# QingYunA/General-Medical-Image-Segmentation-CNN-Framework

Measured on AMD Instinct MI355X. Metric: train voxels/sec (128^3 patches) 3D U-Net, higher is better.
Workload: dtype f32 (f16x3 split MFMA: every fp32 conv operand = two fp16 parts under a per-tensor power-of-two scale, three fp16 products per fp32 product, fp32 accumulate; graded against fp64 by the same tests as bf16x6 and the exact-fp32 MFMA path); 1 GPU; unet3d_f32_2x128: UNet3D(1,2,32) fwd+BCE+bwd+Adam+Dice, x=[2,1,128,128,128] fp32 per GPU, random-init (kaiming) weights, data-parallel replicas with RCCL gradient all-reduce, conv math f16x3; global_batch=2, parallelism=dp1, conv_math=f16x3, optimizer=torch.optim.Adam(fused=True)

## Files before the change

### general-medical-image-segmentation-cnn-framework_amd/csrc/conv_bf16_api.hip

```cpp
#include "common.h"
#include "internal.h"
#include "igemm_kernel.h"

namespace seg {

template <typename TS, typename TD>
__global__ __launch_bounds__(256) void cast_rows_kernel(const TS* __restrict__ src, int lds, TD* __restrict__ dst, int ldd, long long rows, int C) {
    const bool v = (C % 4 == 0) && (lds % 4 == 0) && (ldd % 4 == 0) && ((uintptr_t)src % (4 * sizeof(TS)) == 0) && ((uintptr_t)dst % (4 * sizeof(TD)) == 0);
    const int cw = v ? C / 4 : C;
    const long long total = rows * cw;
    for (long long i = (long long)blockIdx.x * blockDim.x + threadIdx.x; i < total; i += (long long)gridDim.x * blockDim.x) {
        const long long r = i / cw;
        const int c = (int)(i - r * cw);
        if (v) st4(dst + r * ldd + c * 4, ld4(src + r * lds + c * 4));
        else st1(dst + r * ldd + c, ld1(src + r * lds + c));
    }
}

template <typename TS, typename TD>
static void cast_rows(const TS* src, int lds, TD* dst, int ldd, long long rows, int C, hipStream_t st) {
    long long b = (rows * C / 4 + 255) / 256;
    const int grid = (int)(b < 1 ? 1 : (b > 8192 ? 8192 : b));
    hipLaunchKernelGGL((cast_rows_kernel<TS, TD>), dim3(grid), dim3(256), 0, st, src, lds, dst, ldd, rows, C);
}
// ... 35 lines not shown
    {NB_CAST, RUNG(headk_wgrad_supported(SHAPE5(g), g.Cin, g.Cout))},
    {NB_TINY, RUNG(tinypw_supported(SHAPE5(g)))},
    {NB_PWL, RUNG(pointwise(g) && pw_wgrad_lowp_supported(conv_vin(g), g.Cin, g.Cout, k.ldx, k.ldy, 2)), WS(pw_wgrad_lowp_ws_bytes(conv_vin(g), g.Cin, g.Cout)), pointwise, al16, NB_PW},
    {NB_PW, RUNG(pointwise(g) && pw_wgrad_supported(conv_vin(g), g.Cin, g.Cout, 1, k.ldx, k.ldy)), nullptr, nullptr, al8},
    {NB_STEM4, RUNG(stem4_lowp_supported(SHAPE5(g), k.ldx, k.ldy)), ws_stem4, nullptr, al16, NB_STEM},
    {NB_STEM, RUNG(stem_supported(SHAPE5(g), k.ldy)), nullptr, nullptr, al8},
    {NB_HEADPW, RUNG(headpw_lowp_supported(SHAPE5(g), k.ldx, k.ldy)), ws_headpw, nullptr, al16, NB_HEAD},
    {NB_HEAD, RUNG(head_supported(SHAPE5(g), k.ldx)), nullptr, nullptr, al8},
    {NB_SMALLCIN, RUNG(smallcin_wgrad_supported(g.Cin, g.Cout, g.k)), nullptr, nullptr, al8},
    {NB_SMALLCOUT, RUNG(smallcout_wgrad_supported(g.Cin, g.Cout, g.k, k.ldx)), nullptr, nullptr, al8},
    {NB_GW, RUNG(gwgrad_supported(GEOM9(g), k.ldx, k.ldy)), nullptr, nullptr, al8},
    {NB_CAST}};
static int choose_b16(const Rung* r, const ConvKey& k) {
    while (r->fits && !r->fits(k)) ++r;
    if (!r->aligned || r->aligned(k)) return r->family;
    for (const Rung* d = r + 1; r->demote && d->fits; ++d)
        if (d->family == r->demote) return d->fits(k) && d->aligned(k) ? d->family : NB_CAST;
    return NB_CAST;
}

template <typename F>
static int staged(const ConvCall& c, bool x_in, bool y_in, F run) {
    const ConvGeom& g = c.g;
    Carver cv(c.ws);
    float* xf = cv.take<float>((size_t)c.vin() * g.Cin);
    float* yf = cv.take<float>((size_t)c.vout() * g.Cout);
    const size_t used = cv.used();
    SEG_CHECK_WS(used + mi355seg_conv3d_ws_bytes(GEOM9(g)), c.ws_bytes);
    if (x_in) cast_rows((const bf16*)c.x, c.ldx, xf, g.Cin, c.vin(), g.Cin, c.st);
    if (y_in) cast_rows((const bf16*)c.y, c.ldy, yf, g.Cout, c.vout(), g.Cout, c.st);
    SEG_CHECK_LAUNCH();
    int rc = run(xf, yf, (char*)c.ws + used, c.ws_bytes - used);
    if (rc || (x_in && y_in)) return rc;
    if (x_in) cast_rows(yf, g.Cout, (bf16*)c.y, c.ldy, c.vout(), g.Cout, c.st);
    else cast_rows(xf, g.Cin, (bf16*)c.x, c.ldx, c.vin(), g.Cin, c.st);
    SEG_CHECK_LAUNCH();
    return MI355SEG_OK;
}

}

using namespace seg;

extern "C" {

int mi355seg_set_b16_tiles(int mode) {
    SEG_CHECK_ARG(mode >= 0 && mode <= 2, "set_b16_tiles: 0 (auto), 1 (16x16x32 tiles wherever possible) or 2 (generic tiles), got %d", mode);
    set_b16_tiles(mode);
    return MI355SEG_OK;
}
int mi355seg_get_b16_tiles(void) { return get_b16_tiles(); }

int mi355seg_set_wgrad_wide(int mode) {
    SEG_CHECK_ARG(mode >= 0 && mode <= 2, "set_wgrad_wide: 0 (never), 1 (where it pays) or 2 (wherever the geometry allows), got %d", mode);
    set_wgrad_wide(mode);
    return MI355SEG_OK;
}
int mi355seg_get_wgrad_wide(void) { return get_wgrad_wide(); }

size_t mi355seg_conv3d_ws_bytes_bf16(int N, int D, int H, int W, int Cin, int Cout, int k, int stride, int pad) {
    size_t base = mi355seg_conv3d_ws_bytes(N, D, H, W, Cin, Cout, k, stride, pad);
    if (D + 2 * pad < k || H + 2 * pad < k || W + 2 * pad < k) return base;
    const ConvGeom g{N, D, H, W, Cin, Cout, k, stride, pad, (D + 2 * pad - k) / stride + 1, (H + 2 * pad - k) / stride + 1, (W + 2 * pad - k) / stride + 1};
    for (const Rung* ladder : {FWD_B16, DGRAD_B16, WGRAD_B16})
        if (ladder_ws_bytes(ladder, g) > base) base = ladder_ws_bytes(ladder, g);
    const ConvKey d = dense_key(g);
    const bool fb = !choose_b16(FWD_B16, d) || !choose_b16(DGRAD_B16, d) || !choose_b16(WGRAD_B16, d);
    const size_t stage = align_up((size_t)N * D * H * W * Cin * 4, 256) + align_up((size_t)N * g.Do * g.Ho * g.Wo * Cout * 4, 256) + 512;
    if (fb || stage <= ((size_t)512 << 20)) base += stage;
    return base;
}

int mi355seg_conv3d_fused_supported_bf16(int N, int D, int H, int W, int Cin, int Cout, int k, int stride, int pad, int ldx, int ldy) {
    return choose_b16(FWD_B16, ConvKey{{N, D, H, W, Cin, Cout, k, stride, pad, 0, 0, 0}, ldx, ldy, 0, 0, 0}) == NB_IGEMM;
}
int mi355seg_conv3d_fwd_fused_bf16(const mi355seg_bf16* x, int ldx, const float* w, const float* oscale, const float* oshift, int act, float slope,
                                   mi355seg_bf16* y, int ldy, int N, int D, int H, int W, int Cin, int Cout, int k, int stride, int pad,
                                   void* ws, size_t ws_bytes, void* stream) {
    ConvCall c;
    int rc = conv_call(&c, "conv3d_fwd_fused_bf16", x, ldx, w, y, ldy, N, D, H, W, Cin, Cout, k, stride, pad, ws, ws_bytes, stream);
    if (rc) return rc;
    SEG_CHECK_ARG(oscale && oshift, "conv3d_fwd_fused_bf16: null pointer or pitch < channels");
    SEG_CHECK_ARG(choose_b16(FWD_B16, conv_key(c)) == NB_IGEMM, "conv3d_fwd_fused_bf16: no fused form for this shape / alignment (ask mi355seg_conv3d_fused_supported_bf16)");
    MfmaOpts o;
    o.oscale = oscale; o.act = act; o.slope = slope;
    return conv_fwd_mfma(MATH_B16, x, ldx, w, oshift, y, ldy, N, D, H, W, Cin, Cout, k, 0, nullptr, nullptr, ws, ws_bytes, c.st, o);
}

int mi355seg_conv3d_fwd_res_bf16(const mi355seg_bf16* x, int ldx, const float* w, const float* bias, const mi355seg_bf16* res, int ldres,
                                 mi355seg_bf16* y, int ldy, int N, int D, int H, int W, int Cin, int Cout, int k, int stride, int pad,
                                 void* ws, size_t ws_bytes, void* stream) {
    ConvCall c;
    int rc = conv_call(&c, "conv3d_fwd_res_bf16", x, ldx, w, y, ldy, N, D, H, W, Cin, Cout, k, stride, pad, ws, ws_bytes, stream);
    if (rc) return rc;
    SEG_CHECK_ARG(res && ldres >= Cout, "conv3d_fwd_res_bf16: null residual or pitch < channels");
    int fused = 0;
    if (choose_b16(FWD_B16, conv_key(c)) == NB_IGEMM) {
        MfmaOpts o;
        o.res = res; o.ldres = ldres; o.res_fused = &fused;
        rc = conv_fwd_mfma(MATH_B16, x, ldx, w, bias, y, ldy, N, D, H, W, Cin, Cout, k, 0, nullptr, nullptr, ws, ws_bytes, c.st, o);
    } else {
        rc = mi355seg_conv3d_fwd_bf16(x, ldx, w, bias, y, ldy, N, D, H, W, Cin, Cout, k, stride, pad, nullptr, nullptr, ws, ws_bytes, stream);
    }
    if (rc || fused) return rc;
    return mi355seg_act_fwd_bf16(y, ldy, res, ldres, y, ldy, c.vout(), Cout, 0, 0.f, stream);
}

int mi355seg_conv3d_fwd_bf16(const mi355seg_bf16* x, int ldx, const float* w, const float* bias, mi355seg_bf16* y, int ldy,
                             int N, int D, int H, int W, int Cin, int Cout, int k, int stride, int pad,
                             double* stats_sum, double* stats_sq, void* ws, size_t ws_bytes, void* stream) {
    ConvCall c;
// ... 115 lines not shown
```

### general-medical-image-segmentation-cnn-framework_amd/csrc/conv_wgrad_lowp.hip

```cpp
#include "common.h"
#include "internal.h"
#include <initializer_list>
#include <type_traits>
#include <stdlib.h>

namespace seg {

using f32x16 = __attribute__((ext_vector_type(16))) float;
using f32x4 = __attribute__((ext_vector_type(4))) float;
typedef short s16x4 __attribute__((ext_vector_type(4)));
typedef short s16x8 __attribute__((ext_vector_type(8)));
typedef __attribute__((address_space(3))) s16x4 lds_s16x4;

constexpr int LW_WAVES = 8;
constexpr int LW_THREADS = LW_WAVES * 64;
constexpr int LW_TPW = 4;

template <int BX, int KS, int NP, int S = 1>
struct LTile {
    static constexpr int HALO = KS / 2;
    static constexpr int NTAPS = KS == 3 ? 27 : KS * KS;
    static constexpr int PLANES = KS == 3 ? 1 : KS;
    static constexpr int VOX = (NP >= 2 || S == 2) ? 128 : 256;
    static constexpr int TY = BX == 8 ? 8 : 4;
// ... 553 lines not shown
#pragma unroll
                    for (int pr = 0; pr < NPR; ++pr)
#pragma unroll
                        for (int a2 = 0; a2 < 2; ++a2) mfma(cur, tt, a2, b, pr);
                    load_b1(b, ks + 1);
                }
#pragma unroll
                for (int k = 0; k < 4; ++k) { __builtin_amdgcn_sched_group_barrier(0x008, 2 * NPR, 0); __builtin_amdgcn_sched_group_barrier(0x100, 3 * NP, 0); }
            } else {
#pragma unroll
                for (int pr = 0; pr < NPR; ++pr)
#pragma unroll
                    for (int a2 = 0; a2 < 2; ++a2)
#pragma unroll
                        for (int b = 0; b < 4; ++b) mfma(cur, tt, a2, b, pr);
#pragma unroll
                for (int k = 0; k < 8; ++k) { __builtin_amdgcn_sched_group_barrier(0x100, 1, 0); __builtin_amdgcn_sched_group_barrier(0x008, NPR, 0); }
            }
            __builtin_amdgcn_sched_barrier(0);
        }
    };

    int tile = strip;
    tile_geom(tile, tile < a.ntiles);
#pragma unroll
    for (int j = 0; j < NPC; ++j) load_piece(j);
#pragma unroll
    for (int j = 0; j < NPC; ++j) split_piece(j);
    for (; tile < a.ntiles; tile += a.nstrips) {
        __syncthreads();
        if (!LW_DBG(a, 16) || tile == strip) write_stage();
        __syncthreads();
        tile_geom(LW_DBG(a, 64) ? strip : tile + a.nstrips, tile + a.nstrips < a.ntiles && !LW_DBG(a, 8));
        tile_mfma();
    }

#pragma unroll
    for (int tt = 0; tt < FW_TPW; ++tt) {
        const int tap = wave + FW_WAVES * tt;
        float* dst = a.part + (((long long)strip * a.ntaps_total + plane * NTAPS + tap) * a.Cin + ci0 + 4 * g) * a.Cout + co0 + li;
        if (tap <= NTAPS - 1) {
#pragma unroll
            for (int ab = 0; ab < 8; ++ab)
#pragma unroll
                for (int e = 0; e < 4; ++e) {
                    float v = acc[tt][ab >> 2][ab & 3][e];
                    if constexpr (F32) v = __builtin_ldexpf(v, -(sx + sd));
                    dst[(long long)(16 * (ab >> 2) + e) * a.Cout + 16 * (ab & 3)] = v;
                }
        }
    }
}

static int g_wgrad_wide = [] { const char* e = getenv("MI355SEG_WGRAD_WIDE"); return e ? atoi(e) : 1; }();
void set_wgrad_wide(int mode) { g_wgrad_wide = mode; }
int get_wgrad_wide() { return g_wgrad_wide; }

struct LWgradPlan { int KS, BX, ntx, nty, ntz, ntiles, nstrips, npairs, taps, planes, cob; };

static bool lwgrad_plan(int math, int KS, int stride, int N, int D, int H, int W, int Cin, int Cout, LWgradPlan* p, bool wide = false) {
    if ((KS != 3 && KS != 5) || Cin % 32 || Cout % 32 || W < 4) return false;
    if (wide && (stride != 1 || Cout % 64 || (math == MATH_X3 && KS != 3))) return false;
    if (stride != 1 && !(stride == 2 && KS == 3 && math == MATH_B16)) return false;
    const int vox = (math == MATH_X3 || stride == 2) ? 128 : 256;
    int BX = 0; long long best = -1;
    for (int bx : {32, 16, 8}) {
        if (math == MATH_X3 && bx == 32) continue;
        long long padded = (long long)((W + bx - 1) / bx) * bx;
        if (best < 0 || padded < best) { best = padded; BX = bx; }
    }
    const int TY = BX == 8 ? 8 : 4, TZ = (vox / BX) / TY;
    p->KS = KS; p->BX = BX; p->ntx = (W + BX - 1) / BX; p->nty = (H + TY - 1) / TY; p->ntz = (D + TZ - 1) / TZ;
    p->ntiles = N * p->ntz * p->nty * p->ntx;
    p->cob = wide ? 64 : 32;
    p->npairs = (Cin / 32) * (Cout / p->cob);
    p->taps = KS * KS * KS; p->planes = KS == 3 ? 1 : KS;
    const int per_strip = p->npairs * p->planes;
    int want = 256 / per_strip;
    long long cap = (long long)(160u << 20) / ((long long)p->taps * Cin * Cout * 4);
    if (cap < 1) cap = 1;
    if (want > cap) want = (int)cap;
    if (want > p->ntiles) want = p->ntiles;
    if (want < 1) want = 1;
    p->nstrips = want;
    if (wide && g_wgrad_wide != 2 && p->ntiles / p->nstrips < 12) return false;
    return true;
}

static int lw_out(int n, int k, int s, int p) { return (n + 2 * p - k) / s + 1; }

static bool lw_offsets_fit(int math, int H, int W, int ldx, int Ho, int Wo, int lddy) {
    const long long esz = math == MATH_B16 ? 2 : 4;
    return 10ll * (H + 8) * (W + 8) * ldx * esz < 0x7FFF0000ll && 8ll * (Ho + 8) * (Wo + 8) * lddy * esz < 0x7FFF0000ll;
}

bool wgrad_lowp_supported(int math, int N, int D, int H, int W, int Cin, int Cout, int k, int stride, int pad, int ldx, int lddy) {
    const int al = math == MATH_B16 ? 8 : 4;
    if (!((k == 3 && pad == 1) || (k == 5 && pad == 2)) || (ldx % al) || (lddy % al)) return false;
    if (!lw_offsets_fit(math, H, W, ldx, lw_out(H, k, stride, pad), lw_out(W, k, stride, pad), lddy)) return false;
    LWgradPlan p;
    return lwgrad_plan(math, k, stride, N, lw_out(D, k, stride, pad), lw_out(H, k, stride, pad), lw_out(W, k, stride, pad), Cin, Cout, &p);
}

size_t wgrad_lowp_ws_bytes_geom(int N, int D, int H, int W, int Cin, int Cout, int k, int stride, int pad) {
    if (!((k == 3 && pad == 1) || (k == 5 && pad == 2)) || D + 2 * pad < k || H + 2 * pad < k || W + 2 * pad < k) return 0;
    size_t best = 0;
    for (int math : {MATH_X3, MATH_B16}) {
        for (bool wide : {false, true}) {
            LWgradPlan p;
            if (!lwgrad_plan(math, k, stride, N, lw_out(D, k, stride, pad), lw_out(H, k, stride, pad), lw_out(W, k, stride, pad), Cin, Cout, &p, wide)) continue;
            const size_t need = align_up((size_t)p.nstrips * p.taps * Cin * Cout * sizeof(float), 256) + 1024;
            if (need > best) best = need;
        }
    }
    if (k == 3 && stride == 1 && Cin % 64 == 0 && Cout % 64 != 0) {
        LWgradPlan p;
        if (lwgrad_plan(MATH_X3, k, stride, N, lw_out(D, k, stride, pad), lw_out(H, k, stride, pad), lw_out(W, k, stride, pad), Cout, Cin, &p, true)) {
            const size_t need = align_up((size_t)p.nstrips * p.taps * Cin * Cout * sizeof(float), 256) + 1024;
            if (need > best) best = need;
        }
    }
    return best;
}

size_t wgrad_lowp_ws_bytes(int N, int D, int H, int W, int Cin, int Cout, int k) {
    size_t best = 0;
    for (int math : {MATH_X3, MATH_B16}) {
        for (bool wide : {false, true}) {
            LWgradPlan p;
            if (!lwgrad_plan(math, k, 1, N, D, H, W, Cin, Cout, &p, wide)) continue;
            const size_t need = align_up((size_t)p.nstrips * p.taps * Cin * Cout * sizeof(float), 256) + 1024;
            if (need > best) best = need;
        }
    }
    if (k == 3 && Cin % 64 == 0 && Cout % 64 != 0) {
        LWgradPlan p;
        if (lwgrad_plan(MATH_X3, k, 1, N, D, H, W, Cout, Cin, &p, true)) {
            const size_t need = align_up((size_t)p.nstrips * p.taps * Cin * Cout * sizeof(float), 256) + 1024;
            if (need > best) best = need;
        }
    }
    return best;
}

template <int BX, int KS, int NP, typename IN_T, int S = 1>
static void launch_lwgrad(const LWgradArgs& a, int nwg, hipStream_t st) {
    using T = LTile<BX, KS, NP, S>;
    if constexpr (NP == 2 && std::is_same<IN_T, float>::value && S == 1 && KS == 3) {
        if (a.pro_al) {
            SEG_SET_LDS((conv_wgrad_lowp_kernel<BX, KS, NP, IN_T, S, true>), T::LDS_BYTES + 256);
            hipLaunchKernelGGL((conv_wgrad_lowp_kernel<BX, KS, NP, IN_T, S, true>), dim3(nwg), dim3(LW_THREADS), T::LDS_BYTES + 256, st, a);
            return;
        }
    }
    SEG_SET_LDS((conv_wgrad_lowp_kernel<BX, KS, NP, IN_T, S>), T::LDS_BYTES);
    hipLaunchKernelGGL((conv_wgrad_lowp_kernel<BX, KS, NP, IN_T, S>), dim3(nwg), dim3(LW_THREADS), T::LDS_BYTES, st, a);
}

template <int BX, int KS, typename IN_T>
static void launch_wide(const LWgradArgs& a, int nwg, hipStream_t st) {
    using F = FTile<BX, KS, std::is_same<IN_T, float>::value ? 2 : 1>;
    if constexpr (std::is_same<IN_T, float>::value && KS == 3) {
        if (a.pro_al) {
            SEG_SET_LDS((conv_wgrad_wide_kernel<BX, KS, IN_T, true>), F::LDS_BYTES + 256);
            hipLaunchKernelGGL((conv_wgrad_wide_kernel<BX, KS, IN_T, true>), dim3(nwg), dim3(FW_THREADS), F::LDS_BYTES + 256, st, a);
            return;
        }
    }
    SEG_SET_LDS((conv_wgrad_wide_kernel<BX, KS, IN_T>), F::LDS_BYTES);
    hipLaunchKernelGGL((conv_wgrad_wide_kernel<BX, KS, IN_T>), dim3(nwg), dim3(FW_THREADS), F::LDS_BYTES, st, a);
}

template <int KS>
static void dispatch_lwgrad(int math, const LWgradPlan& p, const LWgradArgs& a, int nwg, hipStream_t st) {
    if (math == MATH_X3 && a.amax_x) {
        if (p.BX == 16) launch_lwgrad<16, KS, 2, float>(a, nwg, st);
        else launch_lwgrad<8, KS, 2, float>(a, nwg, st);
    } else if (math == MATH_X3) {
        if (p.BX == 16) launch_lwgrad<16, KS, 3, float>(a, nwg, st);
        else launch_lwgrad<8, KS, 3, float>(a, nwg, st);
    } else {
        if (p.BX == 32) launch_lwgrad<32, KS, 1, bf16>(a, nwg, st);
        else if (p.BX == 16) launch_lwgrad<16, KS, 1, bf16>(a, nwg, st);
        else launch_lwgrad<8, KS, 1, bf16>(a, nwg, st);
    }
}

int conv_wgrad_lowp(int math, const void* dy, int lddy, const void* x, int ldx, float* dw, int N, int D, int H, int W, int Cin,
                    int Cout, int k, int stride, int accumulate, void* ws, size_t ws_bytes, hipStream_t st, const float* x_amax, const float* dy_amax,
                    const ConvPro* pro) {
    LWgradPlan p;
    const int pad = k / 2, Do = lw_out(D, k, stride, pad), Ho = lw_out(H, k, stride, pad), Wo = lw_out(W, k, stride, pad);
    const bool wide = g_wgrad_wide != 0 && (math == MATH_B16 || (math == MATH_X3 && x3_f16())) && lwgrad_plan(math, k, stride, N, Do, Ho, Wo, Cin, Cout, &p, true);
    LWgradPlan psw;
    const bool swap = !wide && !pro && g_wgrad_wide != 0 && math == MATH_X3 && x3_f16() && k == 3 && stride == 1 && Cin % 64 == 0 && Cout % 64 != 0 &&
                      lwgrad_plan(math, k, stride, N, Do, Ho, Wo, Cout, Cin, &psw, true) && psw.nstrips >= 8 && lw_offsets_fit(math, Ho, Wo, lddy, H, W, ldx);
    if (math == MATH_X3) note_conv_path(wide ? MI355SEG_PATH_WGRAD_LOWP_WIDE : (swap ? MI355SEG_PATH_WGRAD_LOWP_SWAPPED : MI355SEG_PATH_WGRAD_LOWP_NARROW));
    if (swap) {
        SEG_CHECK_ARG(((uintptr_t)x % 16) == 0 && ((uintptr_t)dy % 16) == 0, "conv_wgrad_lowp: pointers must be 16-byte aligned");
        Carver cv(ws);
        float* part = cv.take<float>((size_t)psw.nstrips * psw.taps * Cin * Cout);
        float* amax = cv.take<float>(2);
        SEG_CHECK_WS(cv.used(), ws_bytes);
        LWgradArgs a{dy, x, part, lddy, ldx, N, D, H, W, Cout, Cin, Do, Ho, Wo, psw.ntx, psw.nty, psw.ntz, psw.ntiles, psw.nstrips, psw.npairs, Cin / psw.cob, psw.taps,
                     nullptr, nullptr, nullptr, nullptr, 0, 0.f, 0};
        if (!x_amax || !dy_amax) {
            if (hipMemsetAsync(amax, 0, 2 * sizeof(float), st) != hipSuccess) { set_error("conv_wgrad_lowp: hipMemsetAsync failed"); return MI355SEG_EHIP; }
            if (!x_amax) { tensor_amax((const float*)x, ldx, (long long)N * D * H * W, Cin, nullptr, amax, st); x_amax = amax; }
            if (!dy_amax) { tensor_amax((const float*)dy, lddy, (long long)N * Do * Ho * Wo, Cout, nullptr, amax + 1, st); dy_amax = amax + 1; }
            SEG_CHECK_LAUNCH();
        }
        a.amax_x = dy_amax; a.amax_dy = x_amax;
#ifdef MI355SEG_TUNE
        { static const char* e = getenv("MI355SEG_DBG"); a.dbg = e ? atoi(e) : 0; }
#endif
        const int nwg = psw.nstrips * psw.npairs * psw.planes;
        const double vox = (double)N * Do * Ho * Wo;
        {
            ProfScope ps(PF_WGRAD, 2.0 * vox * psw.taps * Cin * Cout, 4.0 * vox * (Cin + Cout) + 4.0 * psw.taps * Cin * Cout, st);
            if (psw.BX == 16) launch_wide<16, 3, float>(a, nwg, st); else launch_wide<8, 3, float>(a, nwg, st);
            SEG_CHECK_LAUNCH();
        }
        wgrad_reduce_swapped(part, dw, psw.nstrips, psw.taps, Cin, Cout, accumulate, st);
        SEG_CHECK_LAUNCH();
        return MI355SEG_OK;
    }
    SEG_CHECK_ARG(wide || lwgrad_plan(math, k, stride, N, Do, Ho, Wo, Cin, Cout, &p), "conv_wgrad_lowp: unsupported shape");
    SEG_CHECK_ARG(((uintptr_t)x % 16) == 0 && ((uintptr_t)dy % 16) == 0, "conv_wgrad_lowp: pointers must be 16-byte aligned");
    SEG_CHECK_ARG(lw_offsets_fit(math, H, W, ldx, Ho, Wo, lddy), "conv_wgrad_lowp: a tile's halo spans more than 2 GB (wgrad_lowp_supported says so)");
    Carver cv(ws);
    float* part = cv.take<float>((size_t)p.nstrips * p.taps * Cin * Cout);
    const bool f16 = math == MATH_X3 && x3_f16();
    float* amax = f16 ? cv.take<float>(2) : nullptr;
    SEG_CHECK_WS(cv.used(), ws_bytes);
    LWgradArgs a{x, dy, part, ldx, lddy, N, D, H, W, Cin, Cout, Do, Ho, Wo, p.ntx, p.nty, p.ntz, p.ntiles, p.nstrips, p.npairs, Cout / p.cob, p.taps, nullptr, nullptr, nullptr, nullptr, 0, 0.f, 0};
    if (f16) {
        if (!x_amax || !dy_amax) {
            if (hipMemsetAsync(amax, 0, 2 * sizeof(float), st) != hipSuccess) { set_error("conv_wgrad_lowp: hipMemsetAsync failed"); return MI355SEG_EHIP; }
            if (!x_amax) { tensor_amax((const float*)x, ldx, (long long)N * D * H * W, Cin, nullptr, amax, st); x_amax = amax; }
            if (!dy_amax) { tensor_amax((const float*)dy, lddy, (long long)N * Do * Ho * Wo, Cout, nullptr, amax + 1, st); dy_amax = amax + 1; }
            SEG_CHECK_LAUNCH();
        }
        a.amax_x = x_amax; a.amax_dy = dy_amax;
    }
    if (pro) {
        SEG_CHECK_ARG(f16 && stride == 1 && k == 3 && pro->al && pro->be && conv_pro_act_ok(pro->act) && x_amax, "conv_wgrad_lowp: the norm + activation prologue needs the f16x3 k3 kernels and the caller's bound on the prologue's output");
        a.pro_al = pro->al; a.pro_be = pro->be; a.pro_act = pro->act; a.pro_slope = pro->act == MI355SEG_ACT_RELU ? 0.f : pro->slope;
        SEG_CHECK_ARG(a.pro_slope >= 0.f && a.pro_slope < 1.f, "conv_wgrad_lowp: prologue slope must lie in [0, 1)");
    }
#ifdef MI355SEG_TUNE
    { static const char* e = getenv("MI355SEG_DBG"); a.dbg = e ? atoi(e) : 0; }
#endif
    const int nwg = p.nstrips * p.npairs * p.planes;
    const double vox = (double)N * Do * Ho * Wo;
    {
        ProfScope ps(PF_WGRAD, 2.0 * vox * p.taps * Cin * Cout, (math == MATH_B16 ? 2.0 : 4.0) * vox * (Cin + Cout) + 4.0 * p.taps * Cin * Cout, st);
        if (wide) {
            if (math == MATH_X3) { if (p.BX == 16) launch_wide<16, 3, float>(a, nwg, st); else launch_wide<8, 3, float>(a, nwg, st); }
            else if (k == 3) { if (p.BX == 32) launch_wide<32, 3, bf16>(a, nwg, st); else if (p.BX == 16) launch_wide<16, 3, bf16>(a, nwg, st); else launch_wide<8, 3, bf16>(a, nwg, st); }
            else { if (p.BX == 32) launch_wide<32, 5, bf16>(a, nwg, st); else if (p.BX == 16) launch_wide<16, 5, bf16>(a, nwg, st); else launch_wide<8, 5, bf16>(a, nwg, st); }
        }
        else if (k == 3 && stride == 2) {
            if (p.BX == 32) launch_lwgrad<32, 3, 1, bf16, 2>(a, nwg, st);
            else if (p.BX == 16) launch_lwgrad<16, 3, 1, bf16, 2>(a, nwg, st);
            else launch_lwgrad<8, 3, 1, bf16, 2>(a, nwg, st);
        }
        else if (k == 3) dispatch_lwgrad<3>(math, p, a, nwg, st);
        else dispatch_lwgrad<5>(math, p, a, nwg, st);
        SEG_CHECK_LAUNCH();
    }
    wgrad_reduce(part, dw, p.nstrips, p.taps, Cin, Cout, accumulate, st);
    SEG_CHECK_LAUNCH();
    return MI355SEG_OK;
}

}
```

### general-medical-image-segmentation-cnn-framework_amd/csrc/igemm_kernel.h

```cpp
#pragma once
#include "common.h"
#include <type_traits>

namespace seg {

using f32x16 = __attribute__((ext_vector_type(16))) float;
using f32x4 = __attribute__((ext_vector_type(4))) float;

#ifdef MI355SEG_TUNE
#define SEG_DBG(a, bit) ((a).dbg & (bit))
#else
#define SEG_DBG(a, bit) 0
#endif

template <int MATH> struct MathTraits;
template <> struct MathTraits<MATH_F32> { using in_t = float; using out_t = float; static constexpr int NP = 1, EPP = 4, LDS_ELEM = 4, KGRAN = 8; };
template <> struct MathTraits<MATH_X3> { using in_t = float; using out_t = float; static constexpr int NP = 3, EPP = 4, LDS_ELEM = 2, KGRAN = 16; };
template <> struct MathTraits<MATH_B16> { using in_t = bf16; using out_t = bf16; static constexpr int NP = 1, EPP = 8, LDS_ELEM = 2, KGRAN = 16; };

template <int MATH, int KS, int BX, int MB, int CK, int WN = 1>
struct Tile {
    using MT = MathTraits<MATH>;
    static constexpr int PITCH = MT::NP * CK + 16 / MT::LDS_ELEM;
    static constexpr int HALO = KS / 2;
// ... 566 lines not shown
    return best;
}

template <int NITER, int NPIECE, int PPV, int HX, int HY, int HZ>
__device__ __forceinline__ void halo_piece_offsets(int (&voff)[NITER], int tid, int ox, int oy, int oz, int D, int H, int W, int bytes_x) {
    constexpr int STEP = 256 / PPV, DZ = STEP / (HY * HX), DY = (STEP % (HY * HX)) / HX, DX = STEP % HX;
    static_assert(256 % PPV == 0 && STEP < 2 * HY * HX, "piece walk: one carry per axis");
    const int sx = bytes_x, sy = W * sx, sz = H * sy;
    const int c1 = DX * sx + DY * sy + DZ * sz, c2 = sy - HX * sx, c3 = sz - HY * sy;
    const int lz = oz < 0 ? -oz : 0, ly = oy < 0 ? -oy : 0, lx = ox < 0 ? -ox : 0;
    const unsigned nz = (unsigned)(min(HZ, D - oz) - lz), ny = (unsigned)(min(HY, H - oy) - ly), nx = (unsigned)(min(HX, W - ox) - lx);
    const int v0 = tid / PPV;
    int hz = v0 / (HY * HX);
    const int rem = v0 - hz * (HY * HX);
    int hy = rem / HX, hx = rem - hy * HX;
    int off = ((oz * H + oy) * W + ox) * sx + hz * sz + hy * sy + hx * sx + (tid % PPV) * 16;
    auto walk = [&](auto BORDER) {
#pragma unroll
        for (int it = 0; it < NITER; ++it) {
            bool ok = true;
            if constexpr (decltype(BORDER)::value) ok = (unsigned)(hz - lz) < nz && (unsigned)(hy - ly) < ny && (unsigned)(hx - lx) < nx;
            if ((it + 1) * 256 > NPIECE) ok = ok && (it * 256 + tid < NPIECE);
            voff[it] = ok ? off : 0x7FFFFFF0;
            hx += DX; off += c1;
            const bool cx = hx >= HX;
            hx -= cx ? HX : 0; hy += cx ? DY + 1 : DY; off += cx ? c2 : 0;
            const bool cy = hy >= HY;
            hy -= cy ? HY : 0; off += cy ? c3 : 0;
            if constexpr (decltype(BORDER)::value) hz += cy ? DZ + 1 : DZ;
        }
    };
    if (ox >= 0 && oy >= 0 && oz >= 0 && ox + HX <= W && oy + HY <= H && oz + HZ <= D) walk(std::false_type{});
    else walk(std::true_type{});
}

constexpr int X3S_NPAIR = 14;
__host__ __device__ constexpr int x3s_pair_tap(int s, int which) {
    if (s < 9) return (s / 3) * 9 + (s % 3) * 3 + which;
    if (s < 12) return (s - 9) * 9 + which * 3 + 2;
    if (s == 12) return which * 9 + 8;
    return which == 0 ? 26 : 27;
}
bool x3s_plan_ok(const IgemmPlan& p, const void* x, int ldx, const void* y, int ldy, long long sample_voxels);
void dispatch_x3s(const IgemmPlan& p, const IgemmArgs& a, int nwg, hipStream_t st);
bool x3w_plan(IgemmPlan& p, int N, int D, int H, int W, int Cin, int Cout, int ksplit);

struct B16sPlan { int KS, WMG, NT, TZ, ntx, nty, ntz, nM, nN, nsteps, ksplit; };
bool b16s_geom(int KS, int N, int D, int H, int W, int Cin, int Cout, B16sPlan* p);
bool b16s_plan(int KS, int N, int D, int H, int W, int Cin, int Cout, const void* x, int ldx, const void* y, int ldy, B16sPlan* p);
size_t b16s_ws_bytes(int N, int D, int H, int W, int Cin, int Cout, int k);
void dispatch_b16s(const B16sPlan& p, const IgemmArgs& a, int nwg, hipStream_t st);
void set_wgrad_wide(int mode);
int get_wgrad_wide();
void set_b16_tiles(int mode);
int get_b16_tiles();

void dispatch_igemm_lowp(int math, const IgemmPlan& p, const IgemmArgs& a, int nwg, hipStream_t st);
bool dispatch_igemm_phases_lowp(int math, const IgemmPlan& p, const IgemmArgs& a, const IgemmPhases& pt, int nwg, hipStream_t st);
bool igemm_lowp_has(int math, int KS, int CK, int BX, int MB);

}
```

### include/mi355seg.h

```cpp
#ifndef MI355SEG_H
#define MI355SEG_H

#include <stddef.h>
#include <stdint.h>

#ifdef __cplusplus
extern "C" {
#endif

#if defined(__HIP__) || defined(__HIPCC__)
typedef __bf16 mi355seg_bf16;
#else
typedef uint16_t mi355seg_bf16;
#endif

#define MI355SEG_OK 0
#define MI355SEG_EINVAL (-1)
#define MI355SEG_EWORKSPACE (-2)
#define MI355SEG_EHIP (-3)

#define MI355SEG_ACT_NONE 0
#define MI355SEG_ACT_RELU 1
#define MI355SEG_ACT_ELU 2
#define MI355SEG_ACT_LRELU 3
#define MI355SEG_ACT_SIGMOID 4

const char* mi355seg_last_error(void);
int mi355seg_version(void);

#define MI355SEG_MATH_FP32 0
#define MI355SEG_MATH_BF16X6 2
#define MI355SEG_MATH_F16X3 3
#define MI355SEG_MATH_DEFAULT MI355SEG_MATH_F16X3
int mi355seg_set_conv_math(int mode);
int mi355seg_get_conv_math(void);
int mi355seg_set_x3_shape(int shape);
int mi355seg_get_x3_shape(void);
int mi355seg_set_b16_tiles(int mode);
int mi355seg_get_b16_tiles(void);
int mi355seg_set_wgrad_wide(int mode);
int mi355seg_get_wgrad_wide(void);

size_t mi355seg_conv3d_ws_bytes(int N, int D, int H, int W, int Cin, int Cout, int k, int stride, int pad);

int mi355seg_conv3d_fwd_f32(const float* x, int ldx, const float* w, const float* bias,
                            float* y, int ldy, int N, int D, int H, int W, int Cin, int Cout,
                            int k, int stride, int pad, double* stats_sum, double* stats_sq,
                            void* ws, size_t ws_bytes, void* stream);

int mi355seg_conv_math_takes_amax(void);
int mi355seg_conv3d_amax_use_f32(int N, int D, int H, int W, int Cin, int Cout, int k, int stride, int pad);
int mi355seg_amax_f32(const float* x, int ld, long long rows, int C, float* amax , void* stream);
int mi355seg_conv3d_fwd_ax_f32(const float* x, int ldx, const float* w, const float* bias,
                               float* y, int ldy, int N, int D, int H, int W, int Cin, int Cout,
                               int k, int stride, int pad, double* stats_sum, double* stats_sq, const float* x_amax, const float* w_amax,
                               void* ws, size_t ws_bytes, void* stream);
int mi355seg_conv3d_dgrad_ax_f32(const float* dy, int lddy, const float* w, float* dx, int lddx,
                                 int N, int D, int H, int W, int Cin, int Cout,
                                 int k, int stride, int pad, const float* dy_amax, const float* w_amax, void* ws, size_t ws_bytes, void* stream);
int mi355seg_conv3d_dgrad_bnsums_ax_f32(const float* dy, int lddy, const float* w, float* dx, int lddx,
                                        int N, int D, int H, int W, int Cin, int Cout, int k, int stride, int pad,
                                        const float* bn_x, int ld_bnx, const float* mean, const float* rstd, const float* gamma, const float* beta,
                                        int act, float slope, float* s1, float* s2, float* dgamma, float* dbeta, const float* dy_amax, const float* w_amax,
                                        void* ws, size_t ws_bytes, void* stream);
int mi355seg_conv3d_wgrad_ax_f32(const float* dy, int lddy, const float* x, int ldx,
                                 float* dw, float* db, int N, int D, int H, int W, int Cin, int Cout,
                                 int k, int stride, int pad, int accumulate, const float* dy_amax, const float* x_amax,
                                 void* ws, size_t ws_bytes, void* stream);

int mi355seg_bn_fold_f32(const float* gamma, const float* beta, const float* mean, const float* var, const float* conv_bias,
                         float eps, int C, float* scale, float* shift, void* stream);
int mi355seg_conv3d_fused_supported_f32(int N, int D, int H, int W, int Cin, int Cout, int k, int stride, int pad, int ldx, int ldy);
int mi355seg_conv3d_fwd_fused_f32(const float* x, int ldx, const float* w, const float* oscale, const float* oshift, int act, float slope,
                                  float* y, int ldy, int N, int D, int H, int W, int Cin, int Cout, int k, int stride, int pad,
                                  void* ws, size_t ws_bytes, void* stream);
int mi355seg_conv3d_fused_supported_bf16(int N, int D, int H, int W, int Cin, int Cout, int k, int stride, int pad, int ldx, int ldy);
int mi355seg_conv3d_fwd_fused_bf16(const mi355seg_bf16* x, int ldx, const float* w, const float* oscale, const float* oshift, int act, float slope,
                                   mi355seg_bf16* y, int ldy, int N, int D, int H, int W, int Cin, int Cout, int k, int stride, int pad,
                                   void* ws, size_t ws_bytes, void* stream);

int mi355seg_conv3d_pro_supported_f32(int N, int D, int H, int W, int Cin, int Cout, int k, int stride, int pad, int act);
int mi355seg_conv3d_fwd_yamax_ax_f32(const float* x, int ldx, const float* w, const float* bias,
                                     float* y, int ldy, int N, int D, int H, int W, int Cin, int Cout,
                                     int k, int stride, int pad, double* stats_sum, double* stats_sq, const float* x_amax, const float* w_amax,
                                     float* y_amax, void* ws, size_t ws_bytes, void* stream);
int mi355seg_norm_fold_f32(const double* sum, const double* sq, long long rows, int C, float eps, const float* gamma, const float* beta, int act,
                           float* mean, float* rstd, float* running_mean, float* running_var, float momentum,
                           const float* x_amax, float* al, float* be, float* a_amax, void* stream);
int mi355seg_conv3d_fwd_pro_ax_f32(const float* x, int ldx, const float* pro_al, const float* pro_be, int pro_act, float pro_slope,
                                   const float* w, const float* bias, float* y, int ldy, int N, int D, int H, int W, int Cin, int Cout,
                                   int k, int stride, int pad, double* stats_sum, double* stats_sq, const float* x_amax, const float* w_amax,
                                   void* ws, size_t ws_bytes, void* stream);
int mi355seg_conv3d_wgrad_pro_ax_f32(const float* dy, int lddy, const float* x, int ldx, const float* pro_al, const float* pro_be, int pro_act, float pro_slope,
                                     float* dw, float* db, int N, int D, int H, int W, int Cin, int Cout,
// ... 387 lines not shown
```

Baseline: 222.4 million voxels/s.

## Add warp-specialized producer/consumer f16x3 wgrad kernel for k3 32x32 convs

Adds a new k3 weight-gradient kernel for the f16x3 path in which four waves run MFMAs while the remaining waves load fp32 x and dy tiles from global memory. The producer waves apply the fused prologue (scale, shift, leaky ReLU), split each value into two fp16 halves and write them into double-buffered LDS. The aim is to overlap global loads and the split work with MFMA compute, which the existing narrow kernel does within the same waves. It is selected by default only for prologue-fused Cin=Cout=32 layers with many tiles per strip; it uses one block per CU and the full LDS, and it adds a query for which wgrad form ran.

```diff
diff --git a/general-medical-image-segmentation-cnn-framework_amd/csrc/conv_bf16_api.hip b/general-medical-image-segmentation-cnn-framework_amd/csrc/conv_bf16_api.hip
--- a/general-medical-image-segmentation-cnn-framework_amd/csrc/conv_bf16_api.hip
+++ b/general-medical-image-segmentation-cnn-framework_amd/csrc/conv_bf16_api.hip
@@ -111,11 +111,12 @@
 int mi355seg_get_b16_tiles(void) { return get_b16_tiles(); }
 
 int mi355seg_set_wgrad_wide(int mode) {
-    SEG_CHECK_ARG(mode >= 0 && mode <= 2, "set_wgrad_wide: 0 (never), 1 (where it pays) or 2 (wherever the geometry allows), got %d", mode);
+    SEG_CHECK_ARG(mode >= 0 && mode <= 3, "set_wgrad_wide: 0 (never), 1 (where it pays), 2 (wide wherever the geometry allows) or 3 (producer / consumer wherever the geometry allows), got %d", mode);
     set_wgrad_wide(mode);
     return MI355SEG_OK;
 }
 int mi355seg_get_wgrad_wide(void) { return get_wgrad_wide(); }
+int mi355seg_last_wgrad_lowp_form(void) { return last_wgrad_lowp_form(); }
 
 size_t mi355seg_conv3d_ws_bytes_bf16(int N, int D, int H, int W, int Cin, int Cout, int k, int stride, int pad) {
     size_t base = mi355seg_conv3d_ws_bytes(N, D, H, W, Cin, Cout, k, stride, pad);
diff --git a/general-medical-image-segmentation-cnn-framework_amd/csrc/conv_wgrad_lowp.hip b/general-medical-image-segmentation-cnn-framework_amd/csrc/conv_wgrad_lowp.hip
--- a/general-medical-image-segmentation-cnn-framework_amd/csrc/conv_wgrad_lowp.hip
+++ b/general-medical-image-segmentation-cnn-framework_amd/csrc/conv_wgrad_lowp.hip
@@ -629,9 +629,266 @@
     }
 }
 
+constexpr int PC_THREADS = 512, PC_CONS = 4, PC_PTHREADS = PC_THREADS - PC_CONS * 64, PC_TPW = 7;
+
+template <int BX, int KS>
+struct PTile {
+    using X = LTile<BX, KS, 2, 1>;
+    static constexpr int ROW = 144;
+    __host__ __device__ static constexpr int row_addr(int v) { return (v >> 1) * (2 * ROW) + (v & 1) * 128; }
+    static constexpr int X_BYTES = X::NVOX * ROW, D_BYTES = X::VOX * ROW, BUF_BYTES = X_BYTES + D_BYTES;
+    static constexpr int LDS_BYTES = 2 * BUF_BYTES;
+    static_assert(LDS_BYTES + 256 <= 160 * 1024, "two tiles and the prologue table do not fit the LDS");
+};
+
+template <int BX, int KS, bool PRO = false>
+__global__ __launch_bounds__(PC_THREADS, 1) void conv_wgrad_pc_kernel(LWgradArgs a) {
+    static_assert(KS == 3, "the producer / consumer form is built for k3");
+    using T = LTile<BX, KS, 2, 1>;
+    using P = PTile<BX, KS>;
+    constexpr int NTAPS = T::NTAPS;
+    extern __shared__ __attribute__((aligned(16))) unsigned char lds[];
+
+    const int tid = threadIdx.x, lane = tid & 63;
+    const int wave = __builtin_amdgcn_readfirstlane(tid >> 6);
+    const int nwg = gridDim.x, bid = blockIdx.x;
+    const int q8 = nwg >> 3, r8 = nwg & 7, xcd = bid & 7;
+    const int t = (xcd < r8 ? xcd * (q8 + 1) : r8 * (q8 + 1) + (xcd - r8) * q8) + (bid >> 3);
+    const int pair = t % a.npairs, strip = t / a.npairs;
+    const int cib = pair / a.ncob, cob = pair % a.ncob;
+    const int ci0 = cib * 32, co0 = cob * 32;
+    const int sx = f16x_scale_exp(*a.amax_x), sd = f16x_scale_exp(*a.amax_dy);
+    float* const ptab = reinterpret_cast<float*>(lds + P::LDS_BYTES);
+    if constexpr (PRO) {
+        const float xscale = pow2f(sx);
+        if (tid < 32) { ptab[tid] = a.pro_al[ci0 + tid] * xscale; ptab[32 + tid] = a.pro_be[ci0 + tid] * xscale; }
+        __syncthreads();
+    }
+
+    if (wave >= PC_CONS) {
+        constexpr int EPP = 4, PPV = 8, ESZ = 4;
+        constexpr int XPIECES = T::NVOX * PPV, DPIECES = T::VOX * PPV;
+        constexpr int XITER = (XPIECES + PC_PTHREADS - 1) / PC_PTHREADS, DITER = DPIECES / PC_PTHREADS;
+        static_assert(DPIECES % PC_PTHREADS == 0, "dy tile must split evenly over the producers");
+        constexpr unsigned OOB = 0x7FFFFFF0u;
+        const int ptid = tid - PC_CONS * 64;
+        const float xscale = pow2f(sx), dscale = pow2f(sd);
+        const float* __restrict__ xin = reinterpret_cast<const float*>(a.x);
+        const float* __restrict__ din = reinterpret_cast<const float*>(a.dy);
+        struct Stage { f32x4 x[XITER], d[DITER]; int xA, xB; };
+        Stage sA, sB;
+        int crd[XITER], rel[XITER], dcrd[DITER], drel[DITER];
+#pragma unroll
+        for (int it = 0; it < XITER; ++it) {
+            const int pc = it * PC_PTHREADS + ptid;
+            const int vox = pc / PPV, part = pc % PPV;
+            const int hz = vox / (T::HY * T::HX), rem = vox % (T::HY * T::HX);
+            const int hy = rem / T::HX, hx = rem % T::HX;
+            crd[it] = pc < XPIECES ? (hx | (hy << 8) | (hz << 16)) : 0x7f7f7f;
+            rel[it] = (((hz * a.H + hy) * a.W + hx) * a.ldx + part * EPP) * ESZ;
+        }
+#pragma unroll
+        for (int it = 0; it < DITER; ++it) {
+            const int pc = it * PC_PTHREADS + ptid;
+            const int vox = pc / PPV, part = pc % PPV;
+            const int line = vox / BX, xx = vox % BX;
+            dcrd[it] = xx | ((line % T::TY) << 8) | ((line / T::TY) << 16);
+            drel[it] = ((((line / T::TY) * a.Ho + line % T::TY) * a.Wo + xx) * a.lddy + part * EPP) * ESZ;
+        }
+        __amdgpu_buffer_rsrc_t rx, rd;
+        int xA = 0, xB = 0, dA = 0;
+        auto clamp7 = [](int v) { return v < 0 ? 0 : (v > 127 ? 127 : v); };
+        auto tile_geom = [&](int tile) {
+            int mt = tile;
+            const int txi = mt % a.ntx; mt /= a.ntx;
+            const int tyi = mt % a.nty; mt /= a.nty;
+            const int tzi = mt % a.ntz;
+            const int n = mt / a.ntz;
+            const int x0 = txi * BX, y0 = tyi * T::TY, z0 = tzi * T::TZ;
+            const int ox = x0 - 1, oy = y0 - 1, oz = z0 - 1;
+            const int lox = clamp7(-ox), loy = clamp7(-oy), loz = clamp7(-oz);
+            const int hix = clamp7(a.W - ox), hiy = clamp7(a.H - oy), hiz = clamp7(a.D - oz);
+            xB = (128 - lox) | ((128 - loy) << 8) | ((128 - loz) << 16);
+            xA = (127 + hix) | ((127 + hiy) << 8) | ((127 + hiz) << 16);
+            dA = (127 + clamp7(a.Wo - x0)) | ((127 + clamp7(a.Ho - y0)) << 8) | ((127 + clamp7(a.Do - z0)) << 16);
+            const float* xb = xin + ((((long long)n * a.D + oz) * a.H + oy) * a.W + ox) * a.ldx + ci0;
+            const float* db = din + ((((long long)n * a.Do + z0) * a.Ho + y0) * a.Wo + x0) * a.lddy + co0;
+            rx = __builtin_amdgcn_make_buffer_rsrc(const_cast<float*>(xb), 0, (int)OOB, 0x00020000);
+            rd = __builtin_amdgcn_make_buffer_rsrc(const_cast<float*>(db), 0, (int)OOB, 0x00020000);
+        };
+        auto x_ok = [&](int it, int bA, int bB) {
+            const int u = bA - crd[it], v = crd[it] + bB;
+            return ((u & v) & 0x808080) == 0x808080;
+        };
+        auto load_tile = [&](Stage& s, int tile) {
+            tile_geom(tile);
+            s.xA = xA; s.xB = xB;
+#pragma unroll
+            for (int it = 0; it < XITER; ++it)
+                s.x[it] = __builtin_bit_cast(f32x4, __builtin_amdgcn_raw_buffer_load_b128(rx, x_ok(it, xA, xB) ? (unsigned)rel[it] : OOB, 0, 0));
+#pragma unroll
+            for (int it = 0; it < DITER; ++it) {
+                const bool ok = ((dA - dcrd[it]) & 0x808080) == 0x808080;
+                s.d[it] = __builtin_bit_cast(f32x4, __builtin_amdgcn_raw_buffer_load_b128(rd, ok ? (unsigned)drel[it] : OOB, 0, 0));
+            }
+        };
+        f32x4 pal = {1.f, 1.f, 1.f, 1.f}, pbe = {0.f, 0.f, 0.f, 0.f};
+        if constexpr (PRO) {
+            pal = *reinterpret_cast<const f32x4*>(ptab + (ptid % PPV) * 4);
+            pbe = *reinterpret_cast<const f32x4*>(ptab + 32 + (ptid % PPV) * 4);
+        }
+        static_assert((PC_PTHREADS / PPV) % 2 == 0 && T::NVOX % 2 == 0, "row pairs");
+        const int prow = P::row_addr(ptid / PPV) + (ptid % PPV) * (EPP * 2);
+        auto put = [&](unsigned char* base, int pc, const f32x4& v, float scale) {
+            unsigned char* dst = base + (pc / PC_PTHREADS) * (PC_PTHREADS / PPV) * P::ROW + prow;
+            f16x4_t qh, ql;
+#pragma unroll
+            for (int e = 0; e < 4; ++e) { _Float16 bh, bl; split2h(v[e] * scale, bh, bl); qh[e] = bh; ql[e] = bl; }
+            *reinterpret_cast<f16x4_t*>(dst) = qh;
+            *reinterpret_cast<f16x4_t*>(dst + 64) = ql;
+        };
+        auto write_tile = [&](const Stage& s, unsigned char* buf) {
+#pragma unroll
+            for (int it = 0; it < XITER; ++it) {
+                const int pc = it * PC_PTHREADS + ptid;
+                if (pc < XPIECES) {
+                    if constexpr (PRO) {
+                        const bool ok = x_ok(it, s.xA, s.xB);
+                        f32x4 z;
+#pragma unroll
+                        for (int e = 0; e < 4; ++e) {
+                            const float tv = fmaf(s.x[it][e], pal[e], pbe[e]);
+                            z[e] = ok ? fmaxf(tv, tv * a.pro_slope) : 0.f;
+                        }
+                        put(buf, pc, z, 1.f);
+                    } else {
+                        put(buf, pc, s.x[it], xscale);
+                    }
+                }
+            }
+#pragma unroll
+            for (int it = 0; it < DITER; ++it) put(buf + P::X_BYTES, it * PC_PTHREADS + ptid, s.d[it], dscale);
+        };
+
+        const int nt = (a.ntiles - strip + a.nstrips - 1) / a.nstrips;
+        auto tile_at = [&](int k) { return strip + k * a.nstrips; };
+#ifdef PC_PRIO
+        __builtin_amdgcn_s_setprio(1);
+#endif
+        load_tile(sA, tile_at(0));
+        if (1 < nt) load_tile(sB, tile_at(1));
+        write_tile(sA, lds);
+        if (2 < nt) load_tile(sA, tile_at(2));
+        __syncthreads();
+        for (int k = 0; k < nt;) {
+            if (k + 1 < nt) {
+                if (!LW_DBG(a, 16)) write_tile(sB, lds + P::BUF_BYTES);
+                if (k + 3 < nt && !LW_DBG(a, 8)) load_tile(sB, tile_at(k + 3));
+            }
+            __syncthreads();
+            if (++k >= nt) break;
+            if (k + 1 < nt) {
+                if (!LW_DBG(a, 16)) write_tile(sA, lds);
+                if (k + 3 < nt && !LW_DBG(a, 8)) load_tile(sA, tile_at(k + 3));
+            }
+            __syncthreads();
+            ++k;
+        }
+    } else {
+        const int li = lane & 15, q = li >> 2, p = li & 3, g = lane >> 4;
+        const int chan_off = 4 * p * 2;
+        static_assert(T::HX % 2 == 0, "line offsets must keep a voxel's parity");
+        const int kq_x = BX == 8 ? (g >> 1) * T::HX + (4 * (g & 1) + q) : (4 * g + q);
+        int dbase = P::X_BYTES + P::row_addr(4 * g + q) + chan_off;
+        int abase[PC_TPW];
+#pragma unroll
+        for (int tt = 0; tt < PC_TPW; ++tt) {
+            int tap = wave + PC_CONS * tt;
+            if (tap > NTAPS - 1) tap = NTAPS - 1;
+            const int dz = tap / 9, dy = (tap / 3) % 3, dx = tap % 3;
+            abase[tt] = ((dz * T::HY + dy) * T::HX + (dx & ~1)) * P::ROW + P::row_addr(kq_x + (dx & 1)) + chan_off;
+        }
+        f32x4 acc[PC_TPW][2][2];
+#pragma unroll
+        for (int tt = 0; tt < PC_TPW; ++tt)
+#pragma unroll
+            for (int ab = 0; ab < 4; ++ab) acc[tt][ab >> 1][ab & 1] = f32x4{0.f, 0.f, 0.f, 0.f};
+
+        auto xoff = [](int ks, int t2) {
+            const int line = BX == 32 ? ks : (BX == 16 ? 2 * ks + t2 : 4 * ks + 2 * t2);
+            return ((((line / T::TY) * T::HY + (line % T::TY)) * T::HX) + (BX == 32 ? 16 * t2 : 0)) * P::ROW;
+        };
+        auto doff = [](int ks, int t2) { return (ks * 32 + 16 * t2) * P::ROW; };
+        auto tile_mfma = [&]() {
+            constexpr int NTT = PC_TPW, NREG = T::KSTEPS * NTT;
+            bf16x8_t bc[2][2], ac[2][2][2];
+            auto load_b = [&](int ks, int b) {
+#pragma unroll
+                for (int pl = 0; pl < 2; ++pl) bc[b][pl] = tr_frag(lds, dbase + doff(ks, 0) + b * 32 + pl * 64, dbase + doff(ks, 1) + b * 32 + pl * 64);
+            };
+            auto load_a = [&](int buf, int ks, int tt) {
+#pragma unroll
+                for (int a2 = 0; a2 < 2; ++a2)
+#pragma unroll
+                    for (int pl = 0; pl < 2; ++pl) ac[buf][a2][pl] = tr_frag(lds, abase[tt] + xoff(ks, 0) + a2 * 32 + pl * 64, abase[tt] + xoff(ks, 1) + a2 * 32 + pl * 64);
+            };
+            auto mfma_half = [&](int cu, int tt, int b) {
+                constexpr int PA[3] = {1, 0, 0}, PB[3] = {0, 1, 0};
+#pragma unroll
+                for (int pr = 0; pr < 3; ++pr)
+#pragma unroll
+                    for (int a2 = 0; a2 < 2; ++a2)
+                        acc[tt][a2][b] = __builtin_amdgcn_mfma_f32_16x16x32_f16(__builtin_bit_cast(f16x8_t, ac[cu][a2][PA[pr]]), __builtin_bit_cast(f16x8_t, bc[b][PB[pr]]),
+                                                                               acc[tt][a2][b], 0, 0, 0);
+            };
+            load_b(0, 0); load_b(0, 1);
+            load_a(0, 0, 0);
+            __builtin_amdgcn_sched_barrier(0);
+#pragma unroll
+            for (int u = 0; u < NREG; ++u) {
+                const int ks = u / NTT, tt = u % NTT, cu = u & 1;
+                if (tt == 0 && ks > 0) load_b(ks, 1);
+                if (u + 1 < NREG) load_a(cu ^ 1, (u + 1) / NTT, (u + 1) % NTT);
+                mfma_half(cu, tt, 0);
+                if (tt == NTT - 1 && ks + 1 < T::KSTEPS) load_b(ks + 1, 0);
+                mfma_half(cu, tt, 1);
+#pragma unroll
+                for (int k = 0; k < 8; ++k) { __builtin_amdgcn_sched_group_barrier(0x100, 2, 0); __builtin_amdgcn_sched_group_barrier(0x008, 1, 0); }
+                __builtin_amdgcn_sched_barrier(0);
+            }
+        };
+
+        int delta = P::BUF_BYTES;
+        __syncthreads();
+        for (int tile = strip; tile < a.ntiles; tile += a.nstrips) {
+            tile_mfma();
+            __syncthreads();
+#pragma unroll
+            for (int tt = 0; tt < PC_TPW; ++tt) abase[tt] += delta;
+            dbase += delta;
+            delta = -delta;
+        }
+
+#pragma unroll
+        for (int tt = 0; tt < PC_TPW; ++tt) {
+            const int tap = wave + PC_CONS * tt;
+            float* dst = a.part + (((long long)strip * a.ntaps_total + tap) * a.Cin + ci0 + 4 * g) * a.Cout + co0 + li;
+            if (tap <= NTAPS - 1) {
+#pragma unroll
+                for (int ab = 0; ab < 4; ++ab)
+#pragma unroll
+                    for (int e = 0; e < 4; ++e)
+                        dst[(long long)(16 * (ab >> 1) + e) * a.Cout + 16 * (ab & 1)] = __builtin_ldexpf(acc[tt][ab >> 1][ab & 1][e], -(sx + sd));
+            }
+        }
+    }
+}
+
 static int g_wgrad_wide = [] { const char* e = getenv("MI355SEG_WGRAD_WIDE"); return e ? atoi(e) : 1; }();
 void set_wgrad_wide(int mode) { g_wgrad_wide = mode; }
 int get_wgrad_wide() { return g_wgrad_wide; }
+static int g_wgrad_lowp_form = 0;
+int last_wgrad_lowp_form() { return g_wgrad_lowp_form; }
 
 struct LWgradPlan { int KS, BX, ntx, nty, ntz, ntiles, nstrips, npairs, taps, planes, cob; };
 
@@ -664,6 +921,8 @@
     return true;
 }
 
+static bool pc_pays(const LWgradPlan& p, int Cin, int Cout, const ConvPro* pro) { return pro && Cin == 32 && Cout == 32 && p.ntiles / p.nstrips >= 64; }
+
 static int lw_out(int n, int k, int s, int p) { return (n + 2 * p - k) / s + 1; }
 
 static bool lw_offsets_fit(int math, int H, int W, int ldx, int Ho, int Wo, int lddy) {
@@ -746,6 +1005,18 @@
     }
     SEG_SET_LDS((conv_wgrad_wide_kernel<BX, KS, IN_T>), F::LDS_BYTES);
     hipLaunchKernelGGL((conv_wgrad_wide_kernel<BX, KS, IN_T>), dim3(nwg), dim3(FW_THREADS), F::LDS_BYTES, st, a);
+}
+
+template <int BX>
+static void launch_pc(const LWgradArgs& a, int nwg, hipStream_t st) {
+    using P = PTile<BX, 3>;
+    if (a.pro_al) {
+        SEG_SET_LDS((conv_wgrad_pc_kernel<BX, 3, true>), P::LDS_BYTES + 256);
+        hipLaunchKernelGGL((conv_wgrad_pc_kernel<BX, 3, true>), dim3(nwg), dim3(PC_THREADS), P::LDS_BYTES + 256, st, a);
+        return;
+    }
+    SEG_SET_LDS((conv_wgrad_pc_kernel<BX, 3>), P::LDS_BYTES);
+    hipLaunchKernelGGL((conv_wgrad_pc_kernel<BX, 3>), dim3(nwg), dim3(PC_THREADS), P::LDS_BYTES, st, a);
 }
 
 template <int KS>
@@ -768,10 +1039,13 @@
                     const ConvPro* pro) {
     LWgradPlan p;
     const int pad = k / 2, Do = lw_out(D, k, stride, pad), Ho = lw_out(H, k, stride, pad), Wo = lw_out(W, k, stride, pad);
-    const bool wide = g_wgrad_wide != 0 && (math == MATH_B16 || (math == MATH_X3 && x3_f16())) && lwgrad_plan(math, k, stride, N, Do, Ho, Wo, Cin, Cout, &p, true);
+    const bool pc = math == MATH_X3 && x3_f16() && k == 3 && stride == 1 && (g_wgrad_wide == 3 || g_wgrad_wide == 1) &&
+                    lwgrad_plan(math, k, stride, N, Do, Ho, Wo, Cin, Cout, &p) && (g_wgrad_wide == 3 || pc_pays(p, Cin, Cout, pro));
+    const bool wide = !pc && g_wgrad_wide != 0 && (math == MATH_B16 || (math == MATH_X3 && x3_f16())) && lwgrad_plan(math, k, stride, N, Do, Ho, Wo, Cin, Cout, &p, true);
     LWgradPlan psw;
-    const bool swap = !wide && !pro && g_wgrad_wide != 0 && math == MATH_X3 && x3_f16() && k == 3 && stride == 1 && Cin % 64 == 0 && Cout % 64 != 0 &&
+    const bool swap = !pc && !wide && !pro && g_wgrad_wide != 0 && math == MATH_X3 && x3_f16() && k == 3 && stride == 1 && Cin % 64 == 0 && Cout % 64 != 0 &&
                       lwgrad_plan(math, k, stride, N, Do, Ho, Wo, Cout, Cin, &psw, true) && psw.nstrips >= 8 && lw_offsets_fit(math, Ho, Wo, lddy, H, W, ldx);
+    g_wgrad_lowp_form = pc ? 3 : (wide ? 1 : (swap ? 2 : 0));
     if (math == MATH_X3) note_conv_path(wide ? MI355SEG_PATH_WGRAD_LOWP_WIDE : (swap ? MI355SEG_PATH_WGRAD_LOWP_SWAPPED : MI355SEG_PATH_WGRAD_LOWP_NARROW));
     if (swap) {
         SEG_CHECK_ARG(((uintptr_t)x % 16) == 0 && ((uintptr_t)dy % 16) == 0, "conv_wgrad_lowp: pointers must be 16-byte aligned");
@@ -802,7 +1076,7 @@
         SEG_CHECK_LAUNCH();
         return MI355SEG_OK;
     }
-    SEG_CHECK_ARG(wide || lwgrad_plan(math, k, stride, N, Do, Ho, Wo, Cin, Cout, &p), "conv_wgrad_lowp: unsupported shape");
+    SEG_CHECK_ARG(wide || pc || lwgrad_plan(math, k, stride, N, Do, Ho, Wo, Cin, Cout, &p), "conv_wgrad_lowp: unsupported shape");
     SEG_CHECK_ARG(((uintptr_t)x % 16) == 0 && ((uintptr_t)dy % 16) == 0, "conv_wgrad_lowp: pointers must be 16-byte aligned");
     SEG_CHECK_ARG(lw_offsets_fit(math, H, W, ldx, Ho, Wo, lddy), "conv_wgrad_lowp: a tile's halo spans more than 2 GB (wgrad_lowp_supported says so)");
     Carver cv(ws);
@@ -832,7 +1106,8 @@
     const double vox = (double)N * Do * Ho * Wo;
     {
         ProfScope ps(PF_WGRAD, 2.0 * vox * p.taps * Cin * Cout, (math == MATH_B16 ? 2.0 : 4.0) * vox * (Cin + Cout) + 4.0 * p.taps * Cin * Cout, st);
-        if (wide) {
+        if (pc) { if (p.BX == 16) launch_pc<16>(a, nwg, st); else launch_pc<8>(a, nwg, st); }
+        else if (wide) {
             if (math == MATH_X3) { if (p.BX == 16) launch_wide<16, 3, float>(a, nwg, st); else launch_wide<8, 3, float>(a, nwg, st); }
             else if (k == 3) { if (p.BX == 32) launch_wide<32, 3, bf16>(a, nwg, st); else if (p.BX == 16) launch_wide<16, 3, bf16>(a, nwg, st); else launch_wide<8, 3, bf16>(a, nwg, st); }
             else { if (p.BX == 32) launch_wide<32, 5, bf16>(a, nwg, st); else if (p.BX == 16) launch_wide<16, 5, bf16>(a, nwg, st); else launch_wide<8, 5, bf16>(a, nwg, st); }
diff --git a/general-medical-image-segmentation-cnn-framework_amd/csrc/igemm_kernel.h b/general-medical-image-segmentation-cnn-framework_amd/csrc/igemm_kernel.h
--- a/general-medical-image-segmentation-cnn-framework_amd/csrc/igemm_kernel.h
+++ b/general-medical-image-segmentation-cnn-framework_amd/csrc/igemm_kernel.h
@@ -642,6 +642,7 @@
 void dispatch_b16s(const B16sPlan& p, const IgemmArgs& a, int nwg, hipStream_t st);
 void set_wgrad_wide(int mode);
 int get_wgrad_wide();
+int last_wgrad_lowp_form();
 void set_b16_tiles(int mode);
 int get_b16_tiles();
 
diff --git a/include/mi355seg.h b/include/mi355seg.h
--- a/include/mi355seg.h
+++ b/include/mi355seg.h
@@ -40,6 +40,7 @@
 int mi355seg_get_b16_tiles(void);
 int mi355seg_set_wgrad_wide(int mode);
 int mi355seg_get_wgrad_wide(void);
+int mi355seg_last_wgrad_lowp_form(void);
 
 size_t mi355seg_conv3d_ws_bytes(int N, int D, int H, int W, int Cin, int Cout, int k, int stride, int pad);
 
```

Measured after the change: 227.4 million voxels/s (median of 6 runs). No clear change (+2.2%).
